# RomanJuranek/librectify

Measured on AMD Instinct MI355X. Metric: Mpix/s end-to-end (detect+VP) on 4K frames, batch call of 64 frames, 5 in flight, higher is better.
Workload: dtype f32

## Files before the change

### librectify_amd/csrc/batch.hip

```cpp
#include "host.h"

#include <cstdio>
#include <cstdlib>
#include <cstring>
#include <string>

namespace lramd {


class LaneSet {
public:
    LaneSet() = default;
    LaneSet(const LaneSet&) = delete;
    LaneSet& operator=(const LaneSet&) = delete;
    int setup(lr_context* caller, int S, bool host_frames, bool keep_workspace) {
        c = caller;
        c->workers.reserve((size_t)std::max(0, S - 1));
        while ((int)c->workers.size() < S - 1) {
            lr_context* wc = nullptr;
            if (ctx_create(c->device, &wc)) return 1;
            c->workers.push_back(wc);
        }
        lanes.reserve((size_t)S);
        lanes.push_back(c);
        for (int i = 0; i < S - 1; ++i) lanes.push_back(c->workers[i]);
        for (lr_context* l : lanes) {
            l->opt = c->opt;
            l->flood_log_min = S == 1 ? 0 : 32;
            l->flood_log_walk = S == 1 ? 0 : 24;
            l->flood_logbig_off = S > 1;
            l->flood_jit_sleep_us = S == 1 ? 0 : 20;
            l->flood_sched_off = true;
            static const bool sleep_env = std::getenv("LIBRECTIFY_LANES_SLEEP") != nullptr;
            l->sleep_in_wait = sleep_env && host_frames;
            l->keep_workspace = keep_workspace;
        }
        return 0;
    }
    ~LaneSet() {
        if (!c) return;
        for (lr_context* l : lanes) {
            l->sleep_in_wait = false;
            l->keep_workspace = false;
            l->flood_sched_off = false;
        }
        c->flood_logbig_off = false;
        c->flood_log_min = c->flood_log_walk = 0;
        c->flood_jit_sleep_us = 0;
    }
    int size() const { return (int)lanes.size(); }
    lr_context* operator[](int i) const { return lanes[(size_t)i]; }

private:
    lr_context* c = nullptr;
    std::vector<lr_context*> lanes;
};

struct BatchOut {
    LineSegment* out;
    int capacity;
    int* n_lines;
    const RectificationConfig* cfg;
    ImageTransform* transforms;
    void write(int b, const std::vector<LineSegment>& res, int w, int h) const {
        const int n = (int)res.size();
        if (n_lines) n_lines[b] = n;
        if (out && capacity > 0 && n > 0) std::memcpy(out + (size_t)b * capacity, res.data(), sizeof(LineSegment) * (size_t)std::min(n, capacity));
        if (transforms) {
            const RectificationConfig def;
            transforms[b] = rectification_transform(res.data(), std::min(n, capacity > 0 ? capacity : n), w, h, cfg ? *cfg : def);
        }
    }
};

template <class Frame>
static int run_lanes(const LaneSet& lanes, int batch, std::atomic<int>& stop, const Frame& frame) {
    const int S = lanes.size();
    std::atomic<int> next_frame{0};
    std::vector<int> rc((size_t)S, 0);
    std::vector<std::string> err((size_t)S);
    auto work = [&](int si) {
        bool failed = false;
        if (si > 0 && hipSetDevice(lanes[0]->device) != hipSuccess) {
            set_error("hipSetDevice failed");
            failed = true;
        }
        while (!failed && !stop.load(std::memory_order_relaxed)) {
            const int b = next_frame.fetch_add(1, std::memory_order_relaxed);
            if (b >= batch) break;
            failed = frame(lanes[si], si, b) != 0;
        }
        if (failed) {
            rc[(size_t)si] = 1;
            err[(size_t)si] = get_error();
            stop.store(1);
        }
    };
    {
        JoinedThreads workers;
        for (int si = 1; si < S; ++si) workers.th.emplace_back(work, si);
        work(0);
    }
    for (int si = 0; si < S; ++si)
        if (rc[(size_t)si]) {
            set_error(err[(size_t)si]);
            return 1;
        }
    return 0;
}

int ctx_find_groups_batch_device(lr_context* c, const void* d_images, int format, size_t image_stride, int batch, int w, int h,
                                 int stride, float min_length, bool refine, LineSegment* out, int capacity, int* n_lines,
                                 const RectificationConfig* cfg, ImageTransform* transforms) {
    if (batch <= 0) return 0;
    const size_t bpp = (size_t)pix_bytes(format);
    if (bpp == 0) {
        set_error("unknown pixel format of the frames");
        return 1;
    }
    LaneSet lanes;
    if (lanes.setup(c, std::max(1, std::min(c->opt.batch_streams, batch)), false, false)) return 1;
    const BatchOut results{out, capacity, n_lines, cfg, transforms};
    std::atomic<int> stop{0};
    return run_lanes(lanes, batch, stop, [&](lr_context* l, int, int b) {
        std::vector<LineSegment> res;
        if (ctx_find_groups_device(l, static_cast<const uint8_t*>(d_images) + (size_t)b * image_stride * bpp, format, w, h, stride, min_length,
                                   refine, res))
            return 1;
        results.write(b, res, w, h);
        return 0;
    });
}

int ctx_find_groups_frames_device(lr_context* c, const lr_frame* frames, int format, bool tagged, int batch, float min_length,
                                  bool refine, LineSegment* out, int capacity, int* n_lines, const RectificationConfig* cfg,
                                  ImageTransform* transforms) {
    auto bad = [](int b, const char* what) {
        set_error("lr_find_line_segment_groups_batch_device: frame " + std::to_string(b) + " of the table: " + what);
        return 1;
    };
    if (pix_bytes(format) == 0) {
        set_error("unknown pixel format of the frames");
        return 1;
    }
    if (frames == nullptr) {
        set_error("lr_find_line_segment_groups_batch_device: no frame table");
        return 1;
    }
    size_t max_pix = 0;
    int max_tiles = 0;
    for (int b = 0; b < batch; ++b) {
        const lr_frame& f = frames[b];
        if (f.data == nullptr) return bad(b, "null data");
        if (f.width < 1 || f.height < 1) return bad(b, "size below 1");
        if (f.stride < f.width) return bad(b, "stride smaller than the width");
        if (format == LR_PIX_F32 && (reinterpret_cast<uintptr_t>(f.data) & 3u)) return bad(b, "f32 address not 4-byte aligned");
        if (f.width < 5 || f.height < 5) {
            if (!tagged) return bad(b, "image smaller than the 5x5 filter");
            continue;
        }
        max_pix = std::max(max_pix, (size_t)f.width * (size_t)f.height);
        max_tiles = std::max(max_tiles, filter_geometry(f.width, f.height).n_tiles);
    }
    LaneSet lanes;
    if (lanes.setup(c, std::max(1, std::min(c->opt.batch_streams, batch)), false, true)) return 1;
    LR_HIP(hipSetDevice(c->device));
    for (int si = 0; si < lanes.size() && max_pix; ++si)
        if (ctx_reserve_workspace(lanes[si], max_pix, max_tiles)) return 1;
    const BatchOut results{out, capacity, n_lines, cfg, transforms};
    std::atomic<int> stop{0};
    return run_lanes(lanes, batch, stop, [&](lr_context* l, int, int b) {
        const lr_frame& f = frames[b];
        std::vector<LineSegment> res;
        if (f.width >= 5 && f.height >= 5 &&
            ctx_find_groups_device(l, f.data, format, f.width, f.height, f.stride, f.min_length < 0.f ? min_length : f.min_length, refine, res))
            return 1;
        results.write(b, res, f.width, f.height);
        return 0;
    });
}

int ctx_find_groups_batch_host(lr_context* c, const void* const* frames, int format, int batch, int w, int h, int stride,
                               float min_length, bool refine, int num_threads, LineSegment* out, int capacity,
                               int* n_lines, const RectificationConfig* cfg, ImageTransform* transforms) {
    if (batch <= 0) return 0;
    const int bpp = pix_bytes(format);
    if (bpp == 0) {
        set_error("unknown pixel format of the frames");
        return 1;
    }
    const int S = std::max(1, std::min(c->opt.batch_streams, batch));
    BatchUploader up(c, frames, batch, w, h, stride, bpp, S, num_threads);
    if (up.check()) return 1;
    LaneSet lanes;
    if (lanes.setup(c, S, true, false) || up.start()) return 1;
    const BatchOut results{out, capacity, n_lines, cfg, transforms};
    const int lanes_rc = run_lanes(lanes, batch, up.stop, [&](lr_context* l, int si, int b) {
        const void* img = nullptr;
        int slot = -1;
        if (up.ready(b, l->stream, &img, &slot)) return 1;
        if (img == nullptr) return 0;
        std::vector<LineSegment> res;
        const double t_f0 = now_ms();
        if (ctx_find_groups_device(l, img, format, w, h, w, min_length, refine, res)) return 1;
        up.release(slot, b, l, si, t_f0);
        results.write(b, res, w, h);
        return 0;
    });
    const std::string& up_err = up.end();
    if (lanes_rc) return 1;
    if (!up_err.empty()) {
        set_error(up_err);
        return 1;
    }
    return 0;
}

int ctx_find_groups_batch_host_multi(lr_context* c, const int* devices, int n_devices, const void* const* frames, int format, int batch,
                                     int w, int h, int stride, float min_length, bool refine, int num_threads,
                                     LineSegment* out, int capacity, int* n_lines, const RectificationConfig* cfg,
                                     ImageTransform* transforms) {
    if (batch <= 0) return 0;
    if (n_devices <= 0 || devices == nullptr) {
        set_error("multi-device batch: empty device list");
        return 1;
    }
    int ndev = 0;
    if (hipGetDeviceCount(&ndev) != hipSuccess) ndev = 0;
    for (int i = 0; i < n_devices; ++i)
        if (devices[i] < 0 || devices[i] >= ndev) {
            set_error("multi-device batch: device index out of range");
            return 1;
        }
    if ((int)c->peers.size() > n_devices) {
        for (size_t i = (size_t)n_devices; i < c->peers.size(); ++i) ctx_destroy(c->peers[i]);
        c->peers.resize((size_t)n_devices);
    }
    c->peers.resize((size_t)n_devices, nullptr);
    for (int i = 0; i < n_devices; ++i) {
        if (c->peers[(size_t)i] && c->peers[(size_t)i]->device != devices[i]) {
            ctx_destroy(c->peers[(size_t)i]);
            c->peers[(size_t)i] = nullptr;
        }
        if (!c->peers[(size_t)i] && ctx_create(devices[i], &c->peers[(size_t)i])) {
            (void)hipSetDevice(c->device);
            return 1;
        }
        c->peers[(size_t)i]->opt = c->opt;
    }
    const int per = (batch + n_devices - 1) / n_devices;
    bool blocks_apart = true;
    if (const size_t fbpp = (size_t)pix_bytes(format)) {
        const size_t span = (size_t)(h - 1) * (size_t)(stride < 0 ? -stride : stride) * fbpp + (size_t)w * fbpp;
        for (int i = 0; i < batch && blocks_apart && w > 0 && h > 0; ++i)
            for (int j = (i / per + 1) * per; j < batch && blocks_apart; ++j) {
                if (!frames[i] || !frames[j]) continue;
                const uintptr_t a = reinterpret_cast<uintptr_t>(frames[i]) - (stride < 0 ? (size_t)(h - 1) * (size_t)(-stride) * fbpp : 0);
                const uintptr_t b = reinterpret_cast<uintptr_t>(frames[j]) - (stride < 0 ? (size_t)(h - 1) * (size_t)(-stride) * fbpp : 0);
                blocks_apart = a + span <= b || b + span <= a;
            }
    }
    for (lr_context* p : c->peers) p->batch_no_register = !blocks_apart;
    std::vector<int> rc((size_t)n_devices, 0);
    std::vector<std::string> err((size_t)n_devices);
    auto run = [&](int i) {
        const int b0 = std::min(batch, i * per), b1 = std::min(batch, b0 + per);
        if (b1 <= b0) return;
        lr_context* p = c->peers[(size_t)i];
        if (hipSetDevice(p->device) != hipSuccess) {
            rc[(size_t)i] = 1;
            err[(size_t)i] = "hipSetDevice failed";
            return;
        }
        const int nt = num_threads > 1 ? std::max(2, num_threads / std::min(n_devices, (batch + per - 1) / per)) : num_threads;
        if (ctx_find_groups_batch_host(p, frames + b0, format, b1 - b0, w, h, stride, min_length, refine, nt,
                                       out ? out + (size_t)b0 * capacity : nullptr, capacity, n_lines ? n_lines + b0 : nullptr, cfg,
                                       transforms ? transforms + b0 : nullptr)) {
            rc[(size_t)i] = 1;
            err[(size_t)i] = get_error();
        }
    };
    std::vector<std::thread> th;
    for (int i = 1; i < n_devices; ++i) th.emplace_back(run, i);
    run(0);
    for (auto& t : th) t.join();
    (void)hipSetDevice(c->device);
    for (int i = 0; i < n_devices; ++i)
        if (rc[(size_t)i]) {
            set_error("device list entry " + std::to_string(i) + " (device " + std::to_string(devices[i]) + "): " + err[(size_t)i]);
            return 1;
        }
    return 0;
}

}
```

### librectify_amd/csrc/host.h

```cpp
#pragma once
#include <atomic>
#include <chrono>
#include <condition_variable>
#include <mutex>
#include <string>
#include <thread>
#include <vector>

#include "context.h"
#include "reg_plan.h"

namespace lramd {

inline double now_ms() {
    return std::chrono::duration<double, std::milli>(std::chrono::steady_clock::now().time_since_epoch()).count();
}

struct JoinedThreads {
    std::vector<std::thread> th;
    void join() {
        for (auto& t : th)
            if (t.joinable()) t.join();
    }
    ~JoinedThreads() { join(); }
};

enum { kCntSeeds = 0, kCntComp = 1, kCntPx = 2, kCntLarge = 4 };

int ensure_flood_buffers(lr_context* c);
int ensure_group_capacity(lr_context* c, size_t n_lines);

int enqueue_groups(lr_context* c, uint32_t line_cap, int max_models, float inlier_deg, float garbage_deg, int n_iter,
                   uint64_t seed, bool model_done = false, bool gather = false);
int run_frame(lr_context* c, const void* d_image, int format, int w, int h, int stride, float min_length, bool refine,
              std::vector<LineSegment>& out, bool filter_enqueued = false);

int ensure_copy_stream(lr_context* c);
bool is_page_locked(const void* p);
int staging_threads(int num_threads, size_t frame_bytes = 0);
void bind_this_thread_near(int device);
int upload_rows(lr_context* c, void* dst, void* stage, const void* buffer, int w, int h, int stride, int bpp, int num_threads,
                hipStream_t up);
int ensure_frame_slot(lr_context* c, int slot, size_t npix, bool pageable, float** stage);
int ensure_upload_ring(lr_context* c, int R, size_t npix, bool staging);

struct StagingCrew {
    lr_context* c = nullptr;
    std::vector<std::thread> th;
    std::atomic<uint32_t> job{0};
    std::atomic<uint64_t> next{0};
    std::atomic<uint64_t> total{0};
    std::atomic<int> bands_left{0}, failed{0};
    std::atomic<bool> quit{false};
    struct Job {
        uint8_t* dst = nullptr;
        uint8_t* stage = nullptr;
        const uint8_t* src = nullptr;
        size_t row_bytes = 0, src_pitch = 0;
        int h = 0, rows_per_band = 1, n_bands = 0;
        hipStream_t up = nullptr;
        int pieces = 1;
        const Event* band_ev = nullptr;
        std::atomic<int>* ready = nullptr;
    } jobs[2];

    static constexpr int kPieces = 8;
    static constexpr int kMaxBands = 256;
    std::atomic<int> pieces_left[2][kMaxBands];

    std::mutex mu;
    std::condition_variable cv;
    std::atomic<int> sleepers{0};
    std::atomic<int> live{0};

    bool work_one(uint32_t gen);
    void work(uint32_t gen) {
        while (work_one(gen)) {
        }
    }
    void start(lr_context* ctx, int helpers);
    int run(void* dst_, void* stage_, const void* buffer, int w_, int h_, int stride_, int bpp_, hipStream_t up_,
            size_t band_bytes = (size_t)4 << 20, int pieces_ = 1) {
        const uint32_t g = begin(dst_, stage_, buffer, w_, h_, stride_, bpp_, up_, nullptr, nullptr, band_bytes, pieces_);
        work(g);
        return finish();
    }
    uint32_t begin(void* dst_, void* stage_, const void* buffer, int w_, int h_, int stride_, int bpp_, hipStream_t up_,
                   const Event* band_ev_, std::atomic<int>* ready_, size_t band_bytes = (size_t)4 << 20, int pieces_ = 0);
    int finish();
    ~StagingCrew();
};

class BatchUploader {
public:
    BatchUploader(lr_context* ctx, const void* const* frames, int batch, int w, int h, int stride, int bpp, int lanes, int num_threads);
    ~BatchUploader();
    BatchUploader(const BatchUploader&) = delete;
    BatchUploader& operator=(const BatchUploader&) = delete;
    int check() const;
    int start();
    int ready(int b, hipStream_t lane_stream, const void** img, int* slot);
    void release(int slot, int b, const lr_context* lane, int lane_index, double t_frame0);
    const std::string& end();
    std::atomic<int> stop{0};

private:
    void close();
    void register_frames();
    void upload_frames();
    int send_frame(StagingCrew& crew, int i, int slot);

    lr_context* c;
    const uint8_t* const* frames;
    const int batch, w, h, stride;
    const size_t bpp, row_bytes, pitch;
    const int lanes, num_threads;
    int R = 0;
    bool any_pageable = false, reg_frames = false, started = false, closed = false;
    std::vector<char> locked;
    std::vector<RegPlan> plan;
    std::vector<std::atomic<int>> enq;
    std::vector<std::atomic<int>> slot_busy;
    struct SlotEdges {
        int r_lo = 0, r_hi = 0;
    };
    std::vector<SlotEdges> slot_edges;
    std::vector<std::atomic<int>> reg_ready;
    std::atomic<int> reg_next{0}, reg_slow{0};
    std::string up_err;
    std::atomic<long long> up_wait_us{0}, lane_wait_us{0}, lead_sum_us{0};
    std::atomic<int> late_frames{0};
    double t_call0 = 0.0;
    JoinedThreads helpers, uploader;
};

}
```

### librectify_amd/csrc/upload.hip

```cpp
#include "host.h"

#include <cstdio>
#include <cstring>
#include <map>
#include <pthread.h>
#include <sched.h>
#if defined(__SSE2__)
#include <immintrin.h>
#endif

static inline void stage_copy(void* dst, const void* src, size_t n) {
#if defined(__SSE2__)
    char* d = static_cast<char*>(dst);
    const char* s_ = static_cast<const char*>(src);
    if (n < 4096) {
        std::memcpy(d, s_, n);
        return;
    }
    const size_t head = (16u - (reinterpret_cast<uintptr_t>(d) & 15u)) & 15u;
    if (head) {
        std::memcpy(d, s_, head);
        d += head;
        s_ += head;
        n -= head;
    }
    size_t blocks = n / 64;
    while (blocks--) {
        const __m128i a = _mm_loadu_si128(reinterpret_cast<const __m128i*>(s_));
        const __m128i b = _mm_loadu_si128(reinterpret_cast<const __m128i*>(s_ + 16));
        const __m128i c2 = _mm_loadu_si128(reinterpret_cast<const __m128i*>(s_ + 32));
        const __m128i e = _mm_loadu_si128(reinterpret_cast<const __m128i*>(s_ + 48));
        _mm_stream_si128(reinterpret_cast<__m128i*>(d), a);
        _mm_stream_si128(reinterpret_cast<__m128i*>(d + 16), b);
        _mm_stream_si128(reinterpret_cast<__m128i*>(d + 32), c2);
        _mm_stream_si128(reinterpret_cast<__m128i*>(d + 48), e);
        s_ += 64;
        d += 64;
    }
    n &= 63;
    if (n) std::memcpy(d, s_, n);
    _mm_sfence();
#else
    std::memcpy(dst, src, n);
#endif
}

namespace lramd {

bool is_page_locked(const void* p) {
    hipPointerAttribute_t a;
    if (hipPointerGetAttributes(&a, p) != hipSuccess) {
        (void)hipGetLastError();
        return false;
    }
    return a.type == hipMemoryTypeHost;
}

int staging_threads(int num_threads, size_t frame_bytes) {
    if (num_threads <= 1) return 1;
    const int hw = (int)std::max(1u, std::thread::hardware_concurrency());
    return std::min(std::min(num_threads, hw), frame_bytes > ((size_t)64 << 20) ? 16 : 8);
}

static std::vector<int> device_node_cpus(int device) {
    static std::mutex mu;
    static std::map<int, std::vector<int>> cache;
    std::lock_guard<std::mutex> lk(mu);
    const auto found = cache.find(device);
    if (found != cache.end()) return found->second;
    std::vector<int>& out = cache[device];
    char bus[64] = {0};
    if (hipDeviceGetPCIBusId(bus, (int)sizeof(bus), device) != hipSuccess) return out;
    for (char* p = bus; *p; ++p) *p = (char)std::tolower((unsigned char)*p);
    int node = -1;
    if (FILE* f = std::fopen((std::string("/sys/bus/pci/devices/") + bus + "/numa_node").c_str(), "r")) {
        if (std::fscanf(f, "%d", &node) != 1) node = -1;
        std::fclose(f);
    }
    if (node < 0) return out;
    char line[4096] = {0};
    if (FILE* f = std::fopen(("/sys/devices/system/node/node" + std::to_string(node) + "/cpulist").c_str(), "r")) {
        if (!std::fgets(line, (int)sizeof(line), f)) line[0] = 0;
        std::fclose(f);
    }
    cpu_set_t allowed;
    CPU_ZERO(&allowed);
    if (sched_getaffinity(0, sizeof(allowed), &allowed) != 0) return out;
    for (const char* p = line; *p;) {
        char* e = nullptr;
        const long a = std::strtol(p, &e, 10);
        if (e == p) break;
        long b = a;
        if (*e == '-') b = std::strtol(e + 1, &e, 10);
        for (long cpu = a; cpu <= b && cpu < CPU_SETSIZE; ++cpu)
            if (CPU_ISSET((int)cpu, &allowed)) out.push_back((int)cpu);
        p = (*e == ',') ? e + 1 : e;
        if (*e != ',') break;
    }
    return out;
}

void bind_this_thread_near(int device) {
    const std::vector<int> cpus = device_node_cpus(device);
    if (cpus.empty()) return;
    cpu_set_t set;
    CPU_ZERO(&set);
    for (int c : cpus) CPU_SET(c, &set);
    (void)pthread_setaffinity_np(pthread_self(), sizeof(set), &set);
}

int ensure_copy_stream(lr_context* c) {
    if (c->copy_stream) return 0;
    LR_HIP(hipSetDevice(c->device));
    int lo = 0, hi = 0;
    if (hipDeviceGetStreamPriorityRange(&lo, &hi) != hipSuccess) lo = hi = 0;
    if (hi == lo) LR_HIP(hipStreamCreateWithFlags(c->copy_stream.put(), hipStreamNonBlocking));
    else LR_HIP(hipStreamCreateWithPriority(c->copy_stream.put(), hipStreamNonBlocking, hi));
    return 0;
}

int upload_rows(lr_context* c, void* dst_, void* stage_, const void* buffer_, int w, int h, int stride, int bpp, int num_threads,
                       hipStream_t up) {
    uint8_t* dst = static_cast<uint8_t*>(dst_);
    uint8_t* stage = static_cast<uint8_t*>(stage_);
    const uint8_t* buffer = static_cast<const uint8_t*>(buffer_);
    if (stride < 0) {
        buffer = buffer + (std::ptrdiff_t)(h - 1) * stride * bpp;
        stride = -stride;
    }
    const size_t row_bytes = (size_t)w * bpp, pitch = (size_t)stride * bpp;
    if (stage == nullptr) {
        if (stride == w)
            LR_HIP(hipMemcpyAsync(dst, buffer, row_bytes * h, hipMemcpyHostToDevice, up));
        else
            LR_HIP(hipMemcpy2DAsync(dst, row_bytes, buffer, pitch, row_bytes, (size_t)h, hipMemcpyHostToDevice, up));
        return 0;
    }
    const int rows_per_band = (int)std::max<size_t>(1, ((size_t)4 << 20) / row_bytes);
    const int n_bands = (h + rows_per_band - 1) / rows_per_band;
    const int T = std::min(staging_threads(num_threads), n_bands);
    std::vector<int> rc(T, 0);
    auto run = [&](int t) {
        if (t > 0 && hipSetDevice(c->device) != hipSuccess) {
            rc[t] = 1;
            return;
        }
        for (int k = t; k < n_bands; k += T) {
            const int r0 = k * rows_per_band, r1 = std::min(h, r0 + rows_per_band);
            if (stride == w) {
                std::memcpy(stage + (size_t)r0 * row_bytes, buffer + (size_t)r0 * pitch, (size_t)(r1 - r0) * row_bytes);
            } else {
                for (int r = r0; r < r1; ++r) std::memcpy(stage + (size_t)r * row_bytes, buffer + (size_t)r * pitch, row_bytes);
            }
            if (hipMemcpyAsync(dst + (size_t)r0 * row_bytes, stage + (size_t)r0 * row_bytes, (size_t)(r1 - r0) * row_bytes,
                               hipMemcpyHostToDevice, up) != hipSuccess)
                rc[t] = 1;
        }
    };
    std::vector<std::thread> th;
    for (int t = 1; t < T; ++t) th.emplace_back(run, t);
    run(0);
    for (auto& x : th) x.join();
    for (int t = 0; t < T; ++t)
        if (rc[t]) {
            (void)hipGetLastError();
            set_error("upload: staging copy failed");
            return 1;
        }
    return 0;
}

bool StagingCrew::work_one(uint32_t gen) {
    for (;;) {
        uint64_t x = next.load(std::memory_order_acquire);
        const uint64_t t = total.load(std::memory_order_acquire);
        if ((uint32_t)(x >> 32) != gen || (uint32_t)(t >> 32) != gen || (uint32_t)x >= (uint32_t)t) return false;
        if (!next.compare_exchange_weak(x, x + 1, std::memory_order_acq_rel)) continue;
        const Job& j = jobs[gen & 1u];
        const size_t row_bytes = j.row_bytes;
        const int kP = j.pieces;
        const int rows_per_piece = (j.rows_per_band + kP - 1) / kP;
        const int k = (int)(uint32_t)x / kP, piece = (int)(uint32_t)x % kP;
        const int b0 = k * j.rows_per_band, b1 = std::min(j.h, b0 + j.rows_per_band);
        const int r0 = std::min(b1, b0 + piece * rows_per_piece), r1 = std::min(b1, r0 + rows_per_piece);
        if (r1 > r0) {
            if (j.src_pitch == row_bytes) {
                stage_copy(j.stage + (size_t)r0 * row_bytes, j.src + (size_t)r0 * j.src_pitch, (size_t)(r1 - r0) * row_bytes);
            } else {
                for (int r = r0; r < r1; ++r) stage_copy(j.stage + (size_t)r * row_bytes, j.src + (size_t)r * j.src_pitch, row_bytes);
            }
        }
        if (pieces_left[gen & 1u][k].fetch_sub(1, std::memory_order_acq_rel) != 1) return true;
        bool ok = hipMemcpyAsync(j.dst + (size_t)b0 * row_bytes, j.stage + (size_t)b0 * row_bytes, (size_t)(b1 - b0) * row_bytes,
                                 hipMemcpyHostToDevice, j.up) == hipSuccess;
        if (ok && j.band_ev) ok = hipEventRecord(j.band_ev[k], j.up) == hipSuccess;
        if (!ok) {
            (void)hipGetLastError();
            failed.store(1);
        }
        if (j.ready) j.ready[k].store(ok ? 1 : -1, std::memory_order_release);
        bands_left.fetch_sub(1, std::memory_order_acq_rel);
        return true;
    }
}

void StagingCrew::start(lr_context* ctx, int helpers) {
    c = ctx;
    live.store(helpers, std::memory_order_relaxed);
    for (int t = 0; t < helpers; ++t)
        th.emplace_back([this]() {
            if (hipSetDevice(c->device) != hipSuccess) {
                (void)hipGetLastError();
                live.fetch_sub(1, std::memory_order_acq_rel);
                return;
            }
            bind_this_thread_near(c->device);
            uint32_t last = 0;
            int spins = 0;
            while (!quit.load(std::memory_order_acquire)) {
                const uint32_t g = job.load(std::memory_order_seq_cst);
                if (g == last) {
                    if (++spins < 512) {
                        std::this_thread::yield();
                        continue;
                    }
                    std::unique_lock<std::mutex> lk(mu);
                    sleepers.fetch_add(1, std::memory_order_seq_cst);
                    cv.wait(lk, [&]() { return quit.load(std::memory_order_acquire) || job.load(std::memory_order_seq_cst) != last; });
                    sleepers.fetch_sub(1, std::memory_order_seq_cst);
                    spins = 0;
                    continue;
                }
                spins = 0;
                last = g;
                work(g);
            }
        });
}

uint32_t StagingCrew::begin(void* dst_, void* stage_, const void* buffer_, int w_, int h_, int stride_, int bpp_, hipStream_t up_,
                            const Event* band_ev_, std::atomic<int>* ready_, size_t band_bytes, int pieces_) {
    const uint8_t* buffer = static_cast<const uint8_t*>(buffer_);
    if (stride_ < 0) {
        buffer = buffer + (std::ptrdiff_t)(h_ - 1) * stride_ * bpp_;
        stride_ = -stride_;
    }
    const uint32_t g = job.load(std::memory_order_relaxed) + 1u;
    Job& j = jobs[g & 1u];
    j.dst = static_cast<uint8_t*>(dst_);
    j.stage = static_cast<uint8_t*>(stage_);
    j.src = buffer;
    j.row_bytes = (size_t)w_ * bpp_;
    j.src_pitch = (size_t)stride_ * bpp_;
    j.h = h_;
    j.up = up_;
    j.band_ev = band_ev_;
    j.ready = ready_;
    j.rows_per_band = (int)std::max<size_t>(1, band_bytes / j.row_bytes);
    j.n_bands = (h_ + j.rows_per_band - 1) / j.rows_per_band;
    if (j.n_bands > kMaxBands) {
        j.rows_per_band = (h_ + kMaxBands - 1) / kMaxBands;
        j.n_bands = (h_ + j.rows_per_band - 1) / j.rows_per_band;
    }
    j.pieces = pieces_ > 0 ? std::min(pieces_, kPieces) : (band_ev_ ? kPieces : 1);
    for (int k = 0; k < j.n_bands; ++k) pieces_left[g & 1u][k].store(j.pieces, std::memory_order_relaxed);
    failed.store(0, std::memory_order_relaxed);
    bands_left.store(j.n_bands, std::memory_order_relaxed);
    total.store(((uint64_t)g << 32) | (uint32_t)(j.n_bands * j.pieces), std::memory_order_release);
    next.store((uint64_t)g << 32, std::memory_order_release);
    job.store(g, std::memory_order_seq_cst);
    if (sleepers.load(std::memory_order_seq_cst) > 0) {
        { std::lock_guard<std::mutex> lk(mu); }
        cv.notify_all();
    }
    return g;
}

int StagingCrew::finish() {
    int spins = 0;
    while (bands_left.load(std::memory_order_acquire) > 0) {
        if (live.load(std::memory_order_acquire) == 0 && work_one(job.load(std::memory_order_relaxed))) continue;
        if (++spins < 256) std::this_thread::yield();
        else std::this_thread::sleep_for(std::chrono::microseconds(10));
    }
    return failed.load() ? 1 : 0;
}

StagingCrew::~StagingCrew() {
    quit.store(true, std::memory_order_seq_cst);
    { std::lock_guard<std::mutex> lk(mu); }
    cv.notify_all();
    for (auto& t : th) t.join();
}

int ensure_frame_slot(lr_context* c, int slot, size_t npix, bool pageable, float** stage) {
    hipStream_t up = c->copy_stream;
    if (c->frames.slot[slot].cap() < npix) {
        LR_HIP(hipStreamSynchronize(c->stream));
        LR_HIP(hipStreamSynchronize(up));
        if (c->frames.slot[slot].grow(npix)) return 1;
    }
    *stage = nullptr;
    if (!pageable) return 0;
    if (c->frames.stage[slot].cap() < npix) {
        LR_HIP(hipStreamSynchronize(up));
        if (c->frames.stage[slot].grow(npix)) return 1;
    }
    LR_HIP(hipEventSynchronize(c->ev_up[slot]));
    *stage = c->frames.stage[slot];
    return 0;
}

int ctx_upload_frame(lr_context* c, int slot, const float* buffer, int w, int h, int stride, int num_threads) {
    LR_HIP(hipSetDevice(c->device));
    if (w < 1 || h < 1 || buffer == nullptr) {
        set_error("upload: bad frame");
        return 1;
    }
    if ((stride < 0 ? -stride : stride) < w) {
        set_error("upload: |stride| smaller than the width");
        return 1;
    }
    if (ensure_copy_stream(c)) return 1;
    float* stage = nullptr;
    if (ensure_frame_slot(c, slot, (size_t)w * h, !is_page_locked(buffer), &stage)) return 1;
    if (upload_rows(c, c->frames.slot[slot], stage, buffer, w, h, stride, (int)sizeof(float), num_threads, c->copy_stream)) return 1;
    LR_HIP(hipEventRecord(c->ev_up[slot], c->copy_stream));
    return 0;
}

int ensure_upload_ring(lr_context* c, int R, size_t npix, bool staging) {
    if (ensure_copy_stream(c)) return 1;
    UploadRing& r = c->ring;
    if ((int)r.img.size() < R || r.cap_pix < npix) {
        LR_HIP(hipStreamSynchronize(c->copy_stream));
        r.cap_pix = 0;
        if ((int)r.img.size() < R) r.img.resize((size_t)R);
        for (auto& b : r.img)
            if (b.grow(npix)) return 1;
        r.cap_pix = npix;
    }
    static const bool lane_debug = std::getenv("LIBRECTIFY_LANE_DEBUG") != nullptr || std::getenv("LIBRECTIFY_BATCH_STATS") != nullptr;
    while (c->ring_ev.size() < r.img.size()) {
        Event e;
        if (e.ensure(lane_debug ? hipEventDefault : hipEventDisableTiming)) return 1;
        c->ring_ev.push_back(std::move(e));
    }
    if (staging && (r.stage.size() < r.img.size() || r.stage_cap_pix < npix)) {
        LR_HIP(hipStreamSynchronize(c->copy_stream));
        r.stage_cap_pix = 0;
        r.stage.resize(r.img.size());
        for (auto& b : r.stage)
            if (b.grow(npix)) return 1;
        r.stage_cap_pix = npix;
    }
    return 0;
}

static bool batch_stats_on() {
    static const bool on = std::getenv("LIBRECTIFY_BATCH_STATS") != nullptr;
    return on;
}
static bool lane_debug_on() {
    static const bool on = std::getenv("LIBRECTIFY_LANE_DEBUG") != nullptr;
    return on;
}
static void nap(int& spins) {
    if (++spins < 64) std::this_thread::yield();
    else std::this_thread::sleep_for(std::chrono::microseconds(30));
}

BatchUploader::BatchUploader(lr_context* ctx, const void* const* frames_, int batch_, int w_, int h_, int stride_, int bpp_, int lanes_,
                             int num_threads_)
    : c(ctx), frames(reinterpret_cast<const uint8_t* const*>(frames_)), batch(batch_), w(w_), h(h_), stride(stride_), bpp((size_t)bpp_),
      row_bytes((size_t)w_ * (size_t)bpp_), pitch((size_t)(stride_ < 0 ? -stride_ : stride_) * (size_t)bpp_), lanes(lanes_),
      num_threads(num_threads_) {}

int BatchUploader::check() const {
    if (w < 1 || h < 1) {
        set_error("upload: bad frame");
        return 1;
    }
    if ((stride < 0 ? -stride : stride) < w) {
        set_error("upload: |stride| smaller than the width");
        return 1;
    }
    for (int i = 0; i < batch; ++i) {
        if (frames[i] == nullptr) {
            set_error("upload: bad frame");
            return 1;
        }
    }
    return 0;
}

int BatchUploader::start() {
    locked.assign((size_t)batch, 0);
    for (int i = 0; i < batch; ++i) {
        locked[(size_t)i] = is_page_locked(frames[i]);
        any_pageable = any_pageable || !locked[(size_t)i];
    }
    static const int extra_env = std::getenv("LIBRECTIFY_RING_EXTRA") ? std::max(1, std::atoi(std::getenv("LIBRECTIFY_RING_EXTRA"))) : 0;
    const size_t npix = (size_t)w * h;
    const int by_bytes = (int)std::min<size_t>(64, ((size_t)2 << 30) / (npix * bpp));
    R = extra_env ? lanes + extra_env : std::max(lanes + 1, std::min(lanes + 6, by_bytes));
    R = std::min(batch, R);
    if (ensure_upload_ring(c, R, npix, any_pageable)) return 1;
    enq = std::vector<std::atomic<int>>((size_t)batch);
    slot_busy = std::vector<std::atomic<int>>((size_t)R);
    slot_edges.assign((size_t)R, SlotEdges());
    for (auto& a : enq) a.store(0, std::memory_order_relaxed);
    for (auto& a : slot_busy) a.store(0, std::memory_order_relaxed);
    static const int register_threads = std::getenv("LIBRECTIFY_REGISTER_FRAMES") ? std::max(0, std::atoi(std::getenv("LIBRECTIFY_REGISTER_FRAMES"))) : 4;
    if (c->register_slow_calls > 0) --c->register_slow_calls;
    reg_frames = register_threads > 0 && any_pageable && stride >= w && c->register_slow_calls == 0;
    if (reg_frames) {
        std::vector<char> may((size_t)batch);
        for (int i = 0; i < batch; ++i) may[(size_t)i] = !locked[(size_t)i] && !c->batch_no_register;
        plan = plan_registrations(reinterpret_cast<const void* const*>(frames), batch, h, pitch, row_bytes, 4096, may.data());
        reg_ready = std::vector<std::atomic<int>>((size_t)batch);
        for (auto& a : reg_ready) a.store(0, std::memory_order_relaxed);
    }
    started = true;
    if (reg_frames)
        for (int t = 0; t < register_threads; ++t) helpers.th.emplace_back([this]() { register_frames(); });
    t_call0 = now_ms();
    uploader.th.emplace_back([this]() { upload_frames(); });
    return 0;
}

void BatchUploader::register_frames() {
    (void)hipSetDevice(c->device);
    bind_this_thread_near(c->device);
    for (int i = reg_next.fetch_add(1, std::memory_order_relaxed); i < batch && !stop.load(std::memory_order_relaxed);
         i = reg_next.fetch_add(1, std::memory_order_relaxed)) {
        if (reg_slow.load(std::memory_order_relaxed) >= 2) break;
        int expect = 0;
        if (!reg_ready[(size_t)i].compare_exchange_strong(expect, 3, std::memory_order_acq_rel)) continue;
        int ok = 2;
        const double t_r0 = now_ms();
        const RegPlan& p = plan[(size_t)i];
        if (p.hi > p.lo)
            ok = hipHostRegister(reinterpret_cast<void*>(p.lo), p.hi - p.lo, hipHostRegisterDefault) == hipSuccess ? 1 : 2;
        if (ok == 2) (void)hipGetLastError();
        if (ok == 1 && (now_ms() - t_r0) * 6.0e6 > (double)(p.hi - p.lo)) reg_slow.fetch_add(1, std::memory_order_relaxed);
        reg_ready[(size_t)i].store(ok, std::memory_order_release);
    }
}

void BatchUploader::upload_frames() {
    if (hipSetDevice(c->device) != hipSuccess) {
        up_err = "hipSetDevice failed";
        stop.store(1);
        return;
    }
    if (any_pageable) bind_this_thread_near(c->device);
    StagingCrew crew;
    if (any_pageable) crew.start(c, staging_threads(num_threads, (size_t)w * h * bpp) - 1);
    for (int i = 0; i < batch; ++i) {
        int slot = -1, spins = 0;
        const double t_w0 = batch_stats_on() ? now_ms() : 0.0;
        while (slot < 0 && !stop.load(std::memory_order_relaxed)) {
            for (int k = 0; k < R && slot < 0; ++k)
                if (!slot_busy[(size_t)k].load(std::memory_order_acquire)) slot = k;
            if (slot < 0) nap(spins);
        }
        if (batch_stats_on()) up_wait_us.fetch_add((long long)((now_ms() - t_w0) * 1e3));
        if (stop.load(std::memory_order_relaxed)) return;
        slot_busy[(size_t)slot].store(1, std::memory_order_relaxed);
        if (reg_frames) {
            int sp2 = 0;
            int expect = 0;
            if (!reg_ready[(size_t)i].compare_exchange_strong(expect, 2, std::memory_order_acq_rel))
                while (reg_ready[(size_t)i].load(std::memory_order_acquire) == 3 && !stop.load(std::memory_order_relaxed)) nap(sp2);
        }
        const double t_u0 = now_ms();
        Event e_dbg;
        if (lane_debug_on() && e_dbg.create() == hipSuccess) (void)hipEventRecord(e_dbg, c->copy_stream);
        if (send_frame(crew, i, slot) || hipEventRecord(c->ring_ev[(size_t)slot], c->copy_stream) != hipSuccess) {
            up_err = get_error().empty() ? "upload failed" : get_error();
            stop.store(1);
            return;
        }
        enq[(size_t)i].store(slot + 1, std::memory_order_release);
        if (lane_debug_on()) {
            const double t_u1 = now_ms();
            float dma = 0.f;
            if (e_dbg) {
                (void)hipEventSynchronize(c->ring_ev[(size_t)slot]);
                if (hipEventElapsedTime(&dma, e_dbg, c->ring_ev[(size_t)slot]) != hipSuccess) (void)hipGetLastError();
            }
            std::fprintf(stderr, "uploader frame %d: slot %d, waited %d naps for it, staged and enqueued in %.2f ms, on the link %.2f ms\n", i, slot, spins, t_u1 - t_u0, dma);
        }
    }
}

int BatchUploader::send_frame(StagingCrew& crew, int i, int slot) {
    constexpr size_t kBatchBand = (size_t)4 << 20;
    const bool registered = reg_frames && reg_ready[(size_t)i].load(std::memory_order_acquire) == 1;
    uint8_t* stage = locked[(size_t)i] ? nullptr : reinterpret_cast<uint8_t*>(c->ring.stage[(size_t)slot].get());
    uint8_t* dimg = reinterpret_cast<uint8_t*>(c->ring.img[(size_t)slot].get());
    if (!registered) {
        slot_edges[(size_t)slot].r_hi = 0;
        return stage ? crew.run(dimg, stage, frames[i], w, h, stride, (int)bpp, c->copy_stream, kBatchBand, 1)
                     : upload_rows(c, dimg, nullptr, frames[i], w, h, stride, (int)bpp, 1, c->copy_stream);
    }
    const RegPlan& p = plan[(size_t)i];
    const uint8_t* f = frames[i];
    for (int r = 0; r < p.r_lo; ++r) std::memcpy(stage + (size_t)r * row_bytes, f + (size_t)r * pitch, row_bytes);
    for (int r = p.r_hi; r < h; ++r) std::memcpy(stage + (size_t)r * row_bytes, f + (size_t)r * pitch, row_bytes);
    slot_edges[(size_t)slot].r_lo = p.r_lo;
    slot_edges[(size_t)slot].r_hi = p.r_hi;
    const hipError_t e = pitch == row_bytes
        ? hipMemcpyAsync(dimg + (size_t)p.r_lo * row_bytes, f + (size_t)p.r_lo * pitch, (size_t)(p.r_hi - p.r_lo) * row_bytes, hipMemcpyHostToDevice, c->copy_stream)
        : hipMemcpy2DAsync(dimg + (size_t)p.r_lo * row_bytes, row_bytes, f + (size_t)p.r_lo * pitch, pitch, row_bytes, (size_t)(p.r_hi - p.r_lo), hipMemcpyHostToDevice, c->copy_stream);
    if (e == hipSuccess) return 0;
    (void)hipGetLastError();
    set_error("upload: transfer of a registered frame failed");
    return 1;
}

int BatchUploader::ready(int b, hipStream_t lane_stream, const void** img, int* slot_out) {
    *img = nullptr;
    int slot = -1, spins = 0;
    const double t_w0 = batch_stats_on() ? now_ms() : 0.0;
    while ((slot = enq[(size_t)b].load(std::memory_order_acquire) - 1) < 0 && !stop.load(std::memory_order_relaxed)) nap(spins);
    if (batch_stats_on()) lane_wait_us.fetch_add((long long)((now_ms() - t_w0) * 1e3));
    if (slot < 0) return 0;
    if (hipStreamWaitEvent(lane_stream, c->ring_ev[(size_t)slot], 0) != hipSuccess) {
        set_error("hipStreamWaitEvent failed");
        return 1;
    }
    uint8_t* dimg = reinterpret_cast<uint8_t*>(c->ring.img[(size_t)slot].get());
    const SlotEdges ed = slot_edges[(size_t)slot];
    if (ed.r_hi > 0) {
        const uint8_t* st = reinterpret_cast<const uint8_t*>(c->ring.stage[(size_t)slot].get());
        hipError_t e = hipSuccess;
        if (ed.r_lo > 0) e = hipMemcpyAsync(dimg, st, (size_t)ed.r_lo * row_bytes, hipMemcpyHostToDevice, lane_stream);
        if (e == hipSuccess && ed.r_hi < h)
            e = hipMemcpyAsync(dimg + (size_t)ed.r_hi * row_bytes, st + (size_t)ed.r_hi * row_bytes, (size_t)(h - ed.r_hi) * row_bytes, hipMemcpyHostToDevice, lane_stream);
        if (e != hipSuccess) {
            (void)hipGetLastError();
            set_error("upload: transfer of a registered frame's first or last rows failed");
            return 1;
        }
    }
    *img = dimg;
    *slot_out = slot;
    return 0;
}

void BatchUploader::release(int slot, int b, const lr_context* l, int lane_index, double t_frame0) {
    if (batch_stats_on() && l->opt.timing_on) {
        float lead = 0.f;
        if (hipEventElapsedTime(&lead, c->ring_ev[(size_t)slot], l->ev[0]) == hipSuccess) {
            lead_sum_us.fetch_add((long long)(lead * 1e3));
            if (lead < 0.05f) late_frames.fetch_add(1);
        } else {
            (void)hipGetLastError();
        }
    }
    if (lane_debug_on()) {
        float lead = 0.f;
        if (hipEventElapsedTime(&lead, c->ring_ev[(size_t)slot], l->ev[0]) != hipSuccess) (void)hipGetLastError();
        std::fprintf(stderr, "lane %d frame %d: enqueue %.2f ms, wait %.2f, whole call %.2f; device total %.2f; upload done %.2f ms before the first kernel\n",
                     lane_index, b, l->host_ms[0], l->host_ms[2], now_ms() - t_frame0, l->stage_ms[LR_T_TOTAL], lead);
    }
    slot_busy[(size_t)slot].store(0, std::memory_order_release);
}

void BatchUploader::close() {
    if (closed || !started) return;
    closed = true;
    uploader.join();
    if (batch_stats_on())
        std::fprintf(stderr, "batch of %d frames: %.2f ms; the uploader waited %.2f ms for free device frames; the %d lanes waited %.2f ms in all for their frame's transfer to be enqueued\n",
                     batch, now_ms() - t_call0, up_wait_us.load() * 1e-3, lanes, lane_wait_us.load() * 1e-3);
    if (batch_stats_on() && c->opt.timing_on)
        std::fprintf(stderr, "   a frame's transfer was finished %.3f ms (mean) before its first kernel started; %d of %d frames started within 0.05 ms of it (they waited for the link)\n",
                     lead_sum_us.load() * 1e-3 / batch, late_frames.load(), batch);
    (void)hipStreamSynchronize(c->copy_stream);
    helpers.join();
    if (reg_slow.load() >= 2) c->register_slow_calls = 32;
    if (reg_frames)
        for (int i = 0; i < batch; ++i)
            if (reg_ready[(size_t)i].load(std::memory_order_acquire) == 1 && hipHostUnregister(reinterpret_cast<void*>(plan[(size_t)i].lo)) != hipSuccess)
                (void)hipGetLastError();
}

const std::string& BatchUploader::end() {
    close();
    return up_err;
}

BatchUploader::~BatchUploader() {
    stop.store(1);
    close();
}

}
```

Baseline: 10620.

## Unregister host frames early on helper threads and start staging crew lazily

```diff
diff --git a/librectify_amd/csrc/batch.hip b/librectify_amd/csrc/batch.hip
--- a/librectify_amd/csrc/batch.hip
+++ b/librectify_amd/csrc/batch.hip
@@ -200,14 +200,18 @@
         int slot = -1;
         if (up.ready(b, l->stream, &img, &slot)) return 1;
         if (img == nullptr) return 0;
+        up.mark_handed(si, b);
         std::vector<LineSegment> res;
         const double t_f0 = now_ms();
         if (ctx_find_groups_device(l, img, format, w, h, w, min_length, refine, res)) return 1;
         up.release(slot, b, l, si, t_f0);
         results.write(b, res, w, h);
+        up.mark_written(b);
         return 0;
     });
+    up.mark_lanes_returned();
     const std::string& up_err = up.end();
+    up.print_account();
     if (lanes_rc) return 1;
     if (!up_err.empty()) {
         set_error(up_err);
diff --git a/librectify_amd/csrc/host.h b/librectify_amd/csrc/host.h
--- a/librectify_amd/csrc/host.h
+++ b/librectify_amd/csrc/host.h
@@ -95,6 +95,10 @@
 public:
     BatchUploader(lr_context* ctx, const void* const* frames, int batch, int w, int h, int stride, int bpp, int lanes, int num_threads);
     ~BatchUploader();
+    void mark_handed(int lane_index, int b);
+    void mark_written(int b);
+    void mark_lanes_returned();
+    void print_account() const;
     BatchUploader(const BatchUploader&) = delete;
     BatchUploader& operator=(const BatchUploader&) = delete;
     int check() const;
@@ -107,6 +111,7 @@
 private:
     void close();
     void register_frames();
+    void release_frames();
     void upload_frames();
     int send_frame(StagingCrew& crew, int i, int slot);
 
@@ -127,10 +132,23 @@
     std::vector<SlotEdges> slot_edges;
     std::vector<std::atomic<int>> reg_ready;
     std::atomic<int> reg_next{0}, reg_slow{0};
+    std::mutex rel_mu;
+    std::condition_variable rel_cv;
+    std::vector<int> rel_q;
+    bool rel_quit = false;
+    std::atomic<int> rel_early{0};
     std::string up_err;
     std::atomic<long long> up_wait_us{0}, lane_wait_us{0}, lead_sum_us{0};
     std::atomic<int> late_frames{0};
     double t_call0 = 0.0;
+    struct Account {
+        double entry = 0.0, crew = -1.0, reg0 = -1.0, enq0 = -1.0, enq_last = -1.0, lanes_back = -1.0, uploader_joined = -1.0,
+               drained = -1.0, helpers_joined = -1.0, unregistered = -1.0;
+        int released_early = 0, released_at_close = 0;
+        std::vector<double> lane_first, start, done, written;
+        std::vector<int> lane_of;
+    } acct;
+    double since_entry() const { return now_ms() - acct.entry; }
     JoinedThreads helpers, uploader;
 };
 
diff --git a/librectify_amd/csrc/upload.hip b/librectify_amd/csrc/upload.hip
--- a/librectify_amd/csrc/upload.hip
+++ b/librectify_amd/csrc/upload.hip
@@ -374,7 +374,9 @@
                              int num_threads_)
     : c(ctx), frames(reinterpret_cast<const uint8_t* const*>(frames_)), batch(batch_), w(w_), h(h_), stride(stride_), bpp((size_t)bpp_),
       row_bytes((size_t)w_ * (size_t)bpp_), pitch((size_t)(stride_ < 0 ? -stride_ : stride_) * (size_t)bpp_), lanes(lanes_),
-      num_threads(num_threads_) {}
+      num_threads(num_threads_) {
+    acct.entry = now_ms();
+}
 
 int BatchUploader::check() const {
     if (w < 1 || h < 1) {
@@ -411,6 +413,11 @@
     slot_edges.assign((size_t)R, SlotEdges());
     for (auto& a : enq) a.store(0, std::memory_order_relaxed);
     for (auto& a : slot_busy) a.store(0, std::memory_order_relaxed);
+    acct.lane_first.assign((size_t)lanes, -1.0);
+    acct.start.assign((size_t)batch, -1.0);
+    acct.done.assign((size_t)batch, -1.0);
+    acct.written.assign((size_t)batch, -1.0);
+    acct.lane_of.assign((size_t)batch, -1);
     static const int register_threads = std::getenv("LIBRECTIFY_REGISTER_FRAMES") ? std::max(0, std::atoi(std::getenv("LIBRECTIFY_REGISTER_FRAMES"))) : 4;
     if (c->register_slow_calls > 0) --c->register_slow_calls;
     reg_frames = register_threads > 0 && any_pageable && stride >= w && c->register_slow_calls == 0;
@@ -446,6 +453,22 @@
         if (ok == 1 && (now_ms() - t_r0) * 6.0e6 > (double)(p.hi - p.lo)) reg_slow.fetch_add(1, std::memory_order_relaxed);
         reg_ready[(size_t)i].store(ok, std::memory_order_release);
     }
+    release_frames();
+}
+
+void BatchUploader::release_frames() {
+    std::unique_lock<std::mutex> lk(rel_mu);
+    for (;;) {
+        rel_cv.wait(lk, [&]() { return !rel_q.empty() || rel_quit; });
+        if (rel_quit) return;
+        const int i = rel_q.back();
+        rel_q.pop_back();
+        lk.unlock();
+        if (hipHostUnregister(reinterpret_cast<void*>(plan[(size_t)i].lo)) != hipSuccess) (void)hipGetLastError();
+        reg_ready[(size_t)i].store(4, std::memory_order_release);
+        rel_early.fetch_add(1, std::memory_order_relaxed);
+        lk.lock();
+    }
 }
 
 void BatchUploader::upload_frames() {
@@ -456,7 +479,6 @@
     }
     if (any_pageable) bind_this_thread_near(c->device);
     StagingCrew crew;
-    if (any_pageable) crew.start(c, staging_threads(num_threads, (size_t)w * h * bpp) - 1);
     for (int i = 0; i < batch; ++i) {
         int slot = -1, spins = 0;
         const double t_w0 = batch_stats_on() ? now_ms() : 0.0;
@@ -475,6 +497,7 @@
                 while (reg_ready[(size_t)i].load(std::memory_order_acquire) == 3 && !stop.load(std::memory_order_relaxed)) nap(sp2);
         }
         const double t_u0 = now_ms();
+        if (i == 0) acct.reg0 = since_entry();
         Event e_dbg;
         if (lane_debug_on() && e_dbg.create() == hipSuccess) (void)hipEventRecord(e_dbg, c->copy_stream);
         if (send_frame(crew, i, slot) || hipEventRecord(c->ring_ev[(size_t)slot], c->copy_stream) != hipSuccess) {
@@ -483,6 +506,8 @@
             return;
         }
         enq[(size_t)i].store(slot + 1, std::memory_order_release);
+        if (i == 0) acct.enq0 = since_entry();
+        if (i == batch - 1) acct.enq_last = since_entry();
         if (lane_debug_on()) {
             const double t_u1 = now_ms();
             float dma = 0.f;
@@ -502,6 +527,10 @@
     uint8_t* dimg = reinterpret_cast<uint8_t*>(c->ring.img[(size_t)slot].get());
     if (!registered) {
         slot_edges[(size_t)slot].r_hi = 0;
+        if (stage && crew.c == nullptr) {
+            crew.start(c, staging_threads(num_threads, (size_t)w * h * bpp) - 1);
+            acct.crew = since_entry();
+        }
         return stage ? crew.run(dimg, stage, frames[i], w, h, stride, (int)bpp, c->copy_stream, kBatchBand, 1)
                      : upload_rows(c, dimg, nullptr, frames[i], w, h, stride, (int)bpp, 1, c->copy_stream);
     }
@@ -566,13 +595,48 @@
         std::fprintf(stderr, "lane %d frame %d: enqueue %.2f ms, wait %.2f, whole call %.2f; device total %.2f; upload done %.2f ms before the first kernel\n",
                      lane_index, b, l->host_ms[0], l->host_ms[2], now_ms() - t_frame0, l->stage_ms[LR_T_TOTAL], lead);
     }
+    acct.done[(size_t)b] = since_entry();
     slot_busy[(size_t)slot].store(0, std::memory_order_release);
+    if (reg_frames && reg_ready[(size_t)b].load(std::memory_order_acquire) == 1) {
+        {
+            std::lock_guard<std::mutex> lk(rel_mu);
+            rel_q.push_back(b);
+        }
+        rel_cv.notify_one();
+    }
+}
+
+void BatchUploader::mark_handed(int lane_index, int b) {
+    const double t = since_entry();
+    if (acct.lane_first[(size_t)lane_index] < 0.0) acct.lane_first[(size_t)lane_index] = t;
+    acct.start[(size_t)b] = t;
+    acct.lane_of[(size_t)b] = lane_index;
+}
+
+void BatchUploader::mark_written(int b) { acct.written[(size_t)b] = since_entry(); }
+
+void BatchUploader::mark_lanes_returned() { acct.lanes_back = since_entry(); }
+
+void BatchUploader::print_account() const {
+    if (!batch_stats_on() || !started) return;
+    const Account& a = acct;
+    std::fprintf(stderr, "account of the call (ms since its entry): crew started %.3f; frame 0 registered %.3f, its transfer enqueued %.3f; last transfer enqueued %.3f\n",
+                 a.crew, a.reg0, a.enq0, a.enq_last);
+    std::fprintf(stderr, "   first frame handed to lane");
+    for (int k = 0; k < lanes; ++k) std::fprintf(stderr, " %d: %.3f", k, a.lane_first[(size_t)k]);
+    std::fprintf(stderr, "\n");
+    for (int b = std::max(0, batch - lanes); b < batch; ++b)
+        std::fprintf(stderr, "   frame %d on lane %d: handed over %.3f, finished %.3f, results written %.3f\n", b, a.lane_of[(size_t)b], a.start[(size_t)b],
+                     a.done[(size_t)b], a.written[(size_t)b]);
+    std::fprintf(stderr, "   lanes returned %.3f; uploader joined %.3f; copy stream drained %.3f; helpers joined %.3f; unregistration done %.3f (%d frames released while the call ran, %d at its end); call returns %.3f\n",
+                 a.lanes_back, a.uploader_joined, a.drained, a.helpers_joined, a.unregistered, a.released_early, a.released_at_close, since_entry());
 }
 
 void BatchUploader::close() {
     if (closed || !started) return;
     closed = true;
     uploader.join();
+    acct.uploader_joined = since_entry();
     if (batch_stats_on())
         std::fprintf(stderr, "batch of %d frames: %.2f ms; the uploader waited %.2f ms for free device frames; the %d lanes waited %.2f ms in all for their frame's transfer to be enqueued\n",
                      batch, now_ms() - t_call0, up_wait_us.load() * 1e-3, lanes, lane_wait_us.load() * 1e-3);
@@ -580,12 +644,24 @@
         std::fprintf(stderr, "   a frame's transfer was finished %.3f ms (mean) before its first kernel started; %d of %d frames started within 0.05 ms of it (they waited for the link)\n",
                      lead_sum_us.load() * 1e-3 / batch, late_frames.load(), batch);
     (void)hipStreamSynchronize(c->copy_stream);
+    acct.drained = since_entry();
+    {
+        std::lock_guard<std::mutex> lk(rel_mu);
+        rel_quit = true;
+    }
+    rel_cv.notify_all();
     helpers.join();
+    acct.released_early = rel_early.load();
+    acct.helpers_joined = since_entry();
     if (reg_slow.load() >= 2) c->register_slow_calls = 32;
     if (reg_frames)
         for (int i = 0; i < batch; ++i)
-            if (reg_ready[(size_t)i].load(std::memory_order_acquire) == 1 && hipHostUnregister(reinterpret_cast<void*>(plan[(size_t)i].lo)) != hipSuccess)
-                (void)hipGetLastError();
+            if (reg_ready[(size_t)i].load(std::memory_order_acquire) == 1) {
+                ++acct.released_at_close;
+                if (hipHostUnregister(reinterpret_cast<void*>(plan[(size_t)i].lo)) != hipSuccess)
+                    (void)hipGetLastError();
+            }
+    acct.unregistered = since_entry();
 }
 
 const std::string& BatchUploader::end() {
```

After: 10670, median of 6. Within noise of the previous version (+0.4%).
